# jviquerat/beacon

Measured on AMD Instinct MI355X. Metric: aggregate env steps/sec, rayleigh-v0 batch=512/GPU 128x64, higher is better.
Workload: dtype f32

## Files before the change

beacon_amd/csrc/jit/ns2d_jit.hip:

```cpp
#if BCN_JIT_ROWS == 1 && BCN_JIT_KIND != 0
#error "ns2d_fast_impl.h (one row per lane, ny <= 64) implements the rayleigh boundary conditions only: mixing needs BCN_JIT_ROWS=2"
#endif
#if BCN_JIT_ROWS == 1
#include "../ns2d_fast_impl.h"
#elif BCN_JIT_ROWS == 2
#include "../ns2d_fast2_impl.h"
#else
#include "../ns2d_fast4_impl.h"
#endif

#ifndef BCN_JIT_GF
#define BCN_JIT_GF 0
#endif

extern "C" {

__attribute__((visibility("default"))) int bcn_jit_launch(const void* args, int batch, void* stream) {
#ifdef BCN_JIT_BREAK
#ifndef BCN_JIT_BREAK_EPS
#define BCN_JIT_BREAK_EPS 3e-4
#endif
  NS2DArgs<BCN_JIT_REAL> a = *static_cast<const NS2DArgs<BCN_JIT_REAL>*>(args);
#if BCN_JIT_BREAK == 2
  a.dt *= BCN_JIT_REAL(1.0 + BCN_JIT_BREAK_EPS);
#else
  a.dt *= BCN_JIT_REAL(1.5);
#endif
#else
  const NS2DArgs<BCN_JIT_REAL>& a = *static_cast<const NS2DArgs<BCN_JIT_REAL>*>(args);
#endif
  if (a.nx != BCN_JIT_NX || a.ny != BCN_JIT_NY || a.kind != BCN_JIT_KIND) {
    bcn_set_error("kernel plugin built for %dx%d kind %d, handle is %dx%d kind %d", BCN_JIT_NX, BCN_JIT_NY, BCN_JIT_KIND,
                  a.nx, a.ny, a.kind);
    return BCN_ERR_ARG;
  }
#if BCN_JIT_ROWS == 1
  return launch_fast<BCN_JIT_REAL, BCN_JIT_NX, BCN_JIT_NY, BCN_JIT_R, BCN_JIT_KIND, BCN_JIT_GF>(a, batch, static_cast<hipStream_t>(stream));
#elif BCN_JIT_ROWS == 2
  return launch_fast2<BCN_JIT_REAL, BCN_JIT_NX, BCN_JIT_NY, BCN_JIT_R, BCN_JIT_KIND, BCN_JIT_GF>(a, batch, static_cast<hipStream_t>(stream));
#else
  return launch_fast4<BCN_JIT_REAL, BCN_JIT_NX, BCN_JIT_NY, BCN_JIT_R, BCN_JIT_RPL, BCN_JIT_KIND>(a, batch, static_cast<hipStream_t>(stream));
#endif
}

__attribute__((visibility("default"))) size_t bcn_jit_scratch_elems(void) {
#if BCN_JIT_ROWS == 1
  return FastGeom<BCN_JIT_NX, BCN_JIT_NY, BCN_JIT_R, BCN_JIT_GF>::scratch_elems();
#elif BCN_JIT_ROWS == 2
  return Fast2Geom<BCN_JIT_NX, BCN_JIT_NY, BCN_JIT_R, BCN_JIT_GF>::scratch_elems();
#else
  return 0;
#endif
}

__attribute__((visibility("default"))) size_t bcn_jit_lds_bytes(void) {
#if BCN_JIT_ROWS == 1
  return FastGeom<BCN_JIT_NX, BCN_JIT_NY, BCN_JIT_R, BCN_JIT_GF>::lds_bytes<BCN_JIT_REAL>();
#elif BCN_JIT_ROWS == 2
  return Fast2Geom<BCN_JIT_NX, BCN_JIT_NY, BCN_JIT_R, BCN_JIT_GF>::lds_elems() * sizeof(BCN_JIT_REAL);
#else
  return (size_t)Fast4Geom<BCN_JIT_NX, BCN_JIT_NY, BCN_JIT_R, BCN_JIT_RPL>::lds_elems(sizeof(BCN_JIT_REAL)) * sizeof(BCN_JIT_REAL);
#endif
}

}
```

beacon_amd/csrc/ns2d_fast_impl.h:

```cpp
#pragma once
#include <stdlib.h>

#include <type_traits>

#include "bcn_dpp.h"
#include "ns2d.h"
#include "ns2d_device.h"
#include "ns2d_sched.h"


#ifndef BCN_R128
#define BCN_R128 16
#endif
#ifndef BCN_R50
#define BCN_R50 5
#endif
#ifndef BCN_GFD
#define BCN_GFD 2
#endif
#ifndef BCN_PDG
#define BCN_PDG 8
#endif
static_assert(BCN_PDG == 4 || BCN_PDG == 8 || BCN_PDG == 10 || BCN_PDG == 12 || BCN_PDG == 16 || BCN_PDG == 20,
              "BCN_PDG: only the prefetch depths that were measured AND verified against the oracle (4, 8, 10, 12, 16, 20)");
#ifndef BCN_PDF
#define BCN_PDF 8
#endif
#ifndef BCN_R128D
#define BCN_R128D 16
#endif



namespace {

using namespace bcn_dpp;

template <int NX, int NY, int R, int GF = 0>
struct FastGeom {
  static_assert(NY <= 64, "lanes run along y");
  static constexpr int NW = (NX + R - 1) / R;
  static constexpr int RL = NX - (NW - 1) * R;
  static_assert(NW <= 16 && RL >= 3 && RL <= R, "at most 16 waves, at least 3 columns each");
  static constexpr int NT = NW * 64;
  static constexpr int SY = NY + 2;
  static constexpr int SX = NX + 2;
  static constexpr int DEADPAD = (GF == 2 && RL != R) ? (R - RL + 2) * SY : 0;
  static constexpr int SZ = (SX * SY + 16 + DEADPAD + 63) / 64 * 64;
  static constexpr int PD = GF ? BCN_PDG : BCN_PDF;
  static constexpr int XC = (GF == 2) ? 2 : 4;
  static constexpr int EXCH = 2 * NW * XC * 64;
  static constexpr int MISC = EXCH + 224 + 16;
  static constexpr int FRONT = ((MISC > 63 * SY + 1 ? MISC : 63 * SY + 1) + 15) / 16 * 16;
  static constexpr int BACK = (NY + 3 * PD + 2) * SY;
  static constexpr int FRONTG = (63 * SY + 1 + 15) / 16 * 16;
  static constexpr int MISCA = (MISC + 15) / 16 * 16;
  static constexpr size_t base_elems() {
    return GF == 1 ? (size_t)MISCA : GF == 2 ? (size_t)MISCA + 2 * (size_t)SZ : (size_t)FRONT + 3 * (size_t)SZ + BACK;
  }
  static constexpr size_t SCR = 3 * (size_t)R * 64;
  template <typename real> static constexpr bool offload() {
    return NW >= 3 && (R + 3) / 4 <= NW - 1 && (base_elems() + SCR) * sizeof(real) <= 160 * 1024;
  }
  template <typename real> static constexpr size_t lds_bytes() {
    return (base_elems() + (offload<real>() ? SCR : 0)) * sizeof(real);
  }
  static constexpr size_t scratch_elems() {
    return GF == 1 ? (size_t)FRONTG + 3 * (size_t)SZ + BACK : GF == 2 ? (size_t)FRONTG + SZ + BACK : 0;
  }
};

typedef float v2f __attribute__((ext_vector_type(2)));
#ifndef BCN_CHAIN_NOP
#define BCN_CHAIN_NOP "s_nop 0\n\t"
#endif
template <int NX, int NY, int R>
__device__ __attribute__((noinline)) void transport_chain_f32(float* Tl, const float* Ul, float* dummy, float c0x, float c1x,
                                                              float c0y, float c1y) {
  using G = FastGeom<NX, NY, R, 0>;
  constexpr int SY = G::SY, PD = G::PD, NSTEP = NX + NY - 1;
  static_assert(PD % 2 == 0, "blocks of an even number of diagonals (packed coefficient fmas)");
  const int lane = threadIdx.x & 63;
  const int j = lane + 1;
  const bool active = lane < NY;
  const int cb = (1 - lane) * SY + j;
  float* Tb = Tl + cb;
  for (int i = 1 + lane; i <= NX; i += 64) Tl[i * SY + 1] += (c0y + c1y * Ul[i * SY + 1 + G::SZ]) * Tl[i * SY];
  float tp = Tl[0 * SY + j];
  float aA[PD], uA[PD], vA[PD], aB[PD], uB[PD], vB[PD];
  typedef __attribute__((address_space(3))) float lds_f;
  lds_f* Tc = (lds_f*)Tb;
  const lds_f* Uc = (const lds_f*)(Ul + cb);
  lds_f* const dummyL = (lds_f*)dummy;
#define BCN_LOAD(RA, RU, RV, OFF)                                                             \
  {                                                                                           \
    const lds_f* const Tq = Tc + (OFF) * SY;                                                  \
    const lds_f* const Uq = Uc + (OFF) * SY;                                                  \
    const lds_f* const Vq = Uq + G::SZ;                                                       \
    _Pragma("unroll") for (int q = 0; q < PD; q++) { RA[q] = Tq[q * SY]; RU[q] = Uq[q * SY]; RV[q] = Vq[q * SY]; } \
  }
#define BCN_BLOCK(RA, RU, RV, NA, NU, NV, OFF, MASK)                                          \
  {                                                                                           \
    BCN_LOAD(NA, NU, NV, (OFF) + PD)                                                          \
    lds_f* const Tq = Tc + (OFF) * SY;                                                        \
    float tq[PD];                                                                             \
    bool okq[PD];                                                                             \
     \
    v2f awp[PD / 2], asp[PD / 2];                                                             \
    _Pragma("unroll") for (int q = 0; q < PD / 2; q++) {                                      \
      const v2f ru = {RU[2 * q], RU[2 * q + 1]}, rv = {RV[2 * q], RV[2 * q + 1]};             \
      awp[q] = c0x + c1x * ru;                                                                \
      asp[q] = c0y + c1y * rv;                                                                \
    }                                                                                         \
    _Pragma("unroll") for (int q = 0; q < PD; q++) {                                          \
      const int t = t0 + (OFF) + q;                                                           \
      const float aw = awp[q / 2][q & 1], as = asp[q / 2][q & 1];                             \
      float t1 = RA[q] + aw * tp;                                                             \
      asm volatile(BCN_CHAIN_NOP "v_fmac_f32_dpp %0, %1, %2 wave_shr:1 row_mask:0xf bank_mask:0xf" \
                   : "+v"(t1) : "v"(tp), "v"(as));                                            \
      okq[q] = (MASK == 0) || (MASK == 4 ? (lane <= t) : (active && (MASK != 2 ? (lane <= t) : true) && \
                               (MASK != 1 ? (lane > t - NX && t < NSTEP) : true)));           \
      tp = okq[q] ? t1 : tp;                                                                  \
                  \
      tq[q] = (MASK == 4 && !okq[q]) ? RA[q] : t1;                                            \
    }                                                                                         \
    if (MASK == 0 || MASK == 4) {                                                             \
      _Pragma("unroll") for (int q = 0; q < PD; q++) Tq[q * SY] = tq[q];                      \
    } else {                                                                                  \
      _Pragma("unroll") for (int q = 0; q < PD; q++) { lds_f* dst = okq[q] ? Tq + q * SY : dummyL; *dst = tq[q]; } \
    }                                                                                         \
  }
#define BCN_CHAIN2(T0, T1, MASK)                                                              \
  _Pragma("nounroll") for (int t0 = (T0); t0 < (T1); t0 += 2 * PD) {                          \
    BCN_BLOCK(aA, uA, vA, aB, uB, vB, 0, MASK)                                                \
    BCN_BLOCK(aB, uB, vB, aA, uA, vA, PD, MASK)                                               \
    Tc += 2 * PD * SY;                                                                        \
    Uc += 2 * PD * SY;                                                                        \
  }
  BCN_LOAD(aA, uA, vA, 0)
  constexpr int P2 = 2 * PD;
  constexpr int TA2 = ((NY - 1 + P2 - 1) / P2) * P2, TB2 = (NX / P2) * P2, TE2 = ((NSTEP + P2 - 1) / P2) * P2;
  if constexpr (TA2 <= TB2 && NY == 64) {
    const float east = Tl[(NX + 1) * SY + j];
    BCN_CHAIN2(0, TA2, 4)
    BCN_CHAIN2(TA2, TE2, 0)
    Tl[(NX + 1) * SY + j] = east;
  } else {
    BCN_CHAIN2(0, TE2, 3)
  }
#undef BCN_CHAIN2
#undef BCN_BLOCK
#undef BCN_LOAD
}

template <typename real, int NX, int NY, int R, int GF>
__device__ __attribute__((noinline)) void transport_chain(real* Tl, const real* Ul, const real* Vl, real* dummy,
                                                          real c0x, real c1x, real c0y, real c1y) {
  using G = FastGeom<NX, NY, R, GF>;
  constexpr int SY = G::SY, PD = G::PD, NSTEP = NX + NY - 1;
  const int lane = threadIdx.x & 63;
  const int j = lane + 1;
  const bool active = lane < NY;
  const int cb = (1 - lane) * SY + j;
  typedef typename std::conditional<GF != 0, __attribute__((address_space(1))) real, __attribute__((address_space(3))) real>::type treal;
  typedef typename std::conditional<GF == 1, __attribute__((address_space(1))) real, __attribute__((address_space(3))) real>::type ureal;
  treal* const Tb = (treal*)(Tl + cb);
  treal* const dummy_t = GF != 0 ? (treal*)(Tl - G::FRONTG) : (treal*)dummy;
  const ureal* const Ug = (const ureal*)Ul;
  const ureal* const Vg = (const ureal*)Vl;
  auto ldu = [&](int t) -> real { const int x = cb + t * SY; return GF == 2 ? Ug[x < 0 ? 0 : (x >= G::SZ ? G::SZ - 1 : x)] : Ug[x]; };
  auto ldv = [&](int t) -> real { const int x = cb + t * SY; return GF == 2 ? Vg[x < 0 ? 0 : (x >= G::SZ ? G::SZ - 1 : x)] : Vg[x]; };
  for (int i = 1 + lane; i <= NX; i += 64) {
    const int x = i * SY + 1;
    ((treal*)Tl)[x] = ((treal*)Tl)[x] + (c0y + c1y * Vg[x]) * ((treal*)Tl)[x - 1];
  }
  asm volatile("s_waitcnt vmcnt(0) lgkmcnt(0)" ::: "memory");
  real ra[PD], ru[PD], rv[PD];
#pragma unroll
  for (int q = 0; q < PD; q++) { ra[q] = Tb[q * SY]; ru[q] = ldu(q); rv[q] = ldv(q); }
  real tp = Tl[0 * SY + j];
#define BCN_CHAIN(T0, T1, MASK)                                                             \
// ... 6 lines not shown
      if (MASK == 0) {                                                                      \
        tp = tn;                                                                            \
        Tb[t * SY] = tn;                                                                    \
      } else {                                                                              \
        const bool ok = active && (MASK != 2 ? (lane <= t) : true) &&                       \
                        (MASK != 1 ? (lane > t - NX && t < NSTEP) : true);                  \
        tp = ok ? tn : tp;                                                                  \
        treal* dst = ok ? Tb + t * SY : dummy_t;                                            \
        *dst = tn;                                                                          \
      }                                                                                     \
      ra[q] = Tb[(t + PD) * SY];                                                            \
      ru[q] = ldu(t + PD);                                                                  \
      rv[q] = ldv(t + PD);                                                                  \
    }                                                                                       \
  }
  constexpr int TA = ((NY - 1 + PD - 1) / PD) * PD;
  constexpr int TB = (NX / PD) * PD;
  if constexpr (TA <= TB) {
    BCN_CHAIN(0, TA, 1)
    if (NY == 64) { BCN_CHAIN(TA, TB, 0) } else { BCN_CHAIN(TA, TB, 1) }
    BCN_CHAIN(TB, NSTEP, 2)
  } else {
    constexpr int TL = ((NY - 1) / PD) * PD, TH = ((NX + PD - 1) / PD) * PD;
    BCN_CHAIN(0, TL, 1)
    BCN_CHAIN(TL, TH, 3)
    BCN_CHAIN(TH, NSTEP, 2)
  }
#undef BCN_CHAIN
}

template <typename real, int NX, int NY, int R0, int RW, int KIND, bool EQ, int GF>
__device__ __forceinline__ void fast_body(const NS2DArgs<real>& A, const int w, const int b, const int it_begin, const int it_end,
                                          const bool first_chunk, const bool last_chunk, char* smem) {
  using G = FastGeom<NX, NY, R0, GF>;
  constexpr int R = RW;
  constexpr int NW = G::NW, NT = G::NT, SY = G::SY, SX = G::SX, SZ = G::SZ, PD = G::PD;
  real* exch = reinterpret_cast<real*>(smem);
  real* errp = exch + G::EXCH;
  real* sact = errp + 128;
  real* red = sact + 64;
  real* gscr = GF ? A.fscr + (size_t)blockIdx.x * A.fscr_stride + G::FRONTG : nullptr;
  real* Ul = GF == 1 ? gscr : GF == 2 ? exch + G::MISCA : exch + G::FRONT;
  real* Vl = Ul + SZ;
  real* Tl = GF == 2 ? gscr : Vl + SZ;

  const int tid = threadIdx.x, lane = tid & 63;
  int j = lane + 1;
  const bool active = lane < NY;
  constexpr int RL = G::RL;
  constexpr bool DEADC = GF == 2 && RW == R0 && RL != R0;
  static_assert(!(DEADC && G::XC == 4), "dead columns exist only in the single-sweep exchange paths (XC == 2, GF == 2)");
  const bool lastw = DEADC && w == NW - 1;
#define LIVE(k) (!DEADC || (k) < RL || !lastw)
  const int i0 = w * R0 + 1;
  const size_t off = (size_t)b * A.ncell;
  real* __restrict__ gu = A.u + off;
  real* __restrict__ gv = A.v + off;
  real* __restrict__ gp = A.p + off;
  real* __restrict__ gS = A.S + off;
  constexpr int XC = G::XC, XL = XC - 1;
  auto exl = [&](int buf, int wave, int which) -> real& { return exch[((buf * NW + wave) * XC + which) * 64 + lane]; };

  for (int c = tid; c < SX * SY; c += NT) {
    const int jj = c / SX, ii = c - jj * SX;
    Ul[ii * SY + jj] = gu[c];
    Vl[ii * SY + jj] = gv[c];
    Tl[ii * SY + jj] = gS[c];
  }
  for (int c = SX * SY + tid; c < SZ; c += NT) { Ul[c] = 0; Vl[c] = 0; Tl[c] = 0; }
  if (tid < 128) errp[tid] = 0;
  real p[R];
#pragma unroll
  for (int k = 0; k < R; k++) p[k] = (active && LIVE(k)) ? gp[j * SX + i0 + k] : real(0);

  if (!first_chunk) {
    if (tid < A.n_sgts) sact[tid] = A.a_last[(size_t)b * A.n_sgts + tid];
  } else {
    const int n = A.n_sgts;
    const real* src = A.actions ? A.actions + (size_t)b * n : A.a_last + (size_t)b * n;
    real mean = 0;
    for (int k = 0; k < n; k++) mean += src[k];
    mean /= (real)n;
    real m = 1;
    for (int k = 0; k < n; k++) {
      real t = bcn_abs(src[k] - mean) / A.C;
      m = t > m ? t : m;
    }
    real mine = (tid < n) ? (src[tid] - mean) / m : real(0);
    __syncthreads();
    if (tid < n) {
      sact[tid] = mine;
      A.a_last[(size_t)b * n + tid] = mine;
      if (A.actions_norm) A.actions_norm[(size_t)b * n + tid] = mine;
    }
  }
  __syncthreads();

  const real dt = A.dt, rdx = A.rdx, rdy = A.rdy, rdx2 = A.rdx2, rdy2 = A.rdy2;
  const real cx = A.cx, cy = A.cy;
  const real wl = active ? real(1) + (j == 1 ? 1 : 0) + ((j == NY && KIND == 0) ? 1 : 0) : real(0);
  const real fW = (active && w == 0) ? real(1) : real(0);
  const real fE = (active && w == NW - 1) ? real(1) : real(0);
// ... 27 lines not shown
  if (tid == 0) {
    slow_k[0] = 0; slow_k[5] = 0;
    slow_k[1] = (real)A.slow_l2lc[0]; slow_k[2] = (real)A.slow_cl[0];
    slow_k[3] = (real)A.slow_l2lc[1]; slow_k[4] = (real)A.slow_cl[1];
  }

  constexpr bool OFFLOAD = G::template offload<real>();
  real* const P0 = exch + G::base_elems();
  real* const US0 = P0 + R0 * 64;
  real* const VX0 = US0 + R0 * 64;
  auto pred = [&](const int i, real uc, real uE_, real uW_, real uN_, real uS_, real uSE_, real vc, real vE_, real vW_, real vN_,
                  real vS_, real vNW_, real pc, real pW, real pS, real& us_out, real& vx_out) {
    {
      real uE = real(0.5) * (uE_ + uc), uW = real(0.5) * (uc + uW_);
      real uN2 = real(0.5) * (uN_ + uc), uS2 = real(0.5) * (uc + uS_);
      real vN2 = real(0.5) * (vN_ + vNW_), vS2 = real(0.5) * (vc + vW_);
      real conv = (uE * uE - uW * uW) * rdx + (uN2 * vN2 - uS2 * vS2) * rdy;
      real diff = ((uE_ - 2 * uc + uW_) * rdx2 + (uN_ - 2 * uc + uS_) * rdy2) * A.kmom;
      real pres = (pc - pW) * rdx;
      us_out = (i >= 2 && (!DEADC || i <= NX) && active) ? uc + dt * (diff - conv - pres) : real(0);
    }
    {
      real vE = real(0.5) * (vE_ + vc), vW = real(0.5) * (vc + vW_);
      real uE = real(0.5) * (uE_ + uSE_), uW = real(0.5) * (uc + uS_);
      real vN2 = real(0.5) * (vN_ + vc), vS2 = real(0.5) * (vc + vS_);
      real conv = (uE * vE - uW * vW) * rdx + (vN2 * vN2 - vS2 * vS2) * rdy;
      real diff = ((vE_ - 2 * vc + vW_) * rdx2 + (vN_ - 2 * vc + vS_) * rdy2) * A.kmom;
      real pres = (pc - pS) * rdy;
      vx_out = diff - conv - pres;
    }
  };
  auto bc_uv = [&]() {
    for (int jj = 1 + tid; jj <= NY; jj += NT) {
      Ul[1 * SY + jj] = 0;
      Ul[(NX + 1) * SY + jj] = 0;
      if (jj >= 2) {
        Vl[0 * SY + jj] = -Vl[1 * SY + jj];
        Vl[(NX + 1) * SY + jj] = -Vl[NX * SY + jj];
      }
    }
    for (int ii = 1 + tid; ii <= NX + 1; ii += NT) {
      const bool wall = (ii == 1) || (ii == NX + 1);
      const real utop = wall ? real(0) : Ul[ii * SY + NY];
      const real ubot = wall ? real(0) : Ul[ii * SY + 1];
      Ul[ii * SY + NY + 1] = -utop;
      Ul[ii * SY + 0] = -ubot;
      if (ii <= NX) {
        Vl[ii * SY + NY + 1] = 0;
        Vl[ii * SY + 1] = 0;
      }
    }
  };
  auto publish_p = [&]() {
    exl(xb, w, 1) = p[R - 1];
    if (OFFLOAD && w == 0) {
#pragma unroll
      for (int k = 0; k < R; k++) P0[k * 64 + lane] = p[k];
    }
  };

  bc_uv();
  publish_p();
  __syncthreads();

  real us[R], vs[R];
  for (int it = it_begin;; it++) {
    asm volatile("" : "+v"(j));
    const bool have_chain = it > it_begin;
    const bool have_pred = it < it_end && status == 0;
    real vx[R];
    const bool pred_own = have_pred && (w != 0 || !have_chain);
    if (w == 0 && have_chain) {
#ifndef BCN_CHAIN_PRIO
#define BCN_CHAIN_PRIO 3
#endif
      __builtin_amdgcn_s_setprio(BCN_CHAIN_PRIO);
      if constexpr (std::is_same<real, float>::value && GF == 0)
        transport_chain_f32<NX, NY, R0>(Tl, Ul, red + 16, dt * A.ksc * rdx2, real(0.5) * dt * rdx, dt * A.ksc * rdy2,
                                        real(0.5) * dt * rdy);
      else
        transport_chain<real, NX, NY, R0, GF>(Tl, Ul, Vl, red + 16, dt * A.ksc * rdx2, real(0.5) * dt * rdx,
                                              dt * A.ksc * rdy2, real(0.5) * dt * rdy);
      __builtin_amdgcn_s_setprio(0);
      BCN_PH(6)
    }
#define BCN_OWN_PRED                                                                                            \
    {                                                                                                           \
      const real pWh = (w > 0) ? exl(xb, w - 1, 1) : real(0);                                              \
       \
      constexpr bool WIDE = (R > 16) || (R > 12 && NW > 8);    \
      constexpr int CH = GF ? 4 : (!WIDE ? R : (R % 4 == 0 ? 4 : 5));    \
      _Pragma("unroll") for (int c0 = 0; c0 < R; c0 += CH) {                                                    \
        if (CH != R) __builtin_amdgcn_sched_barrier(0);           \
        real ur[CH + 2], uS[CH + 1], uN[CH], vr[CH + 2], vN[CH + 1], vS[CH];                                    \
        const int ic = i0 + c0;                                                                                 \
        _Pragma("unroll") for (int k = 0; k < CH + 2; k++) { ur[k] = Ul[(ic - 1 + k) * SY + j]; vr[k] = Vl[(ic - 1 + k) * SY + j]; } \
        _Pragma("unroll") for (int k = 0; k < CH + 1; k++) { uS[k] = Ul[(ic + k) * SY + j - 1]; vN[k] = Vl[(ic - 1 + k) * SY + j + 1]; } \
        _Pragma("unroll") for (int k = 0; k < CH; k++) { uN[k] = Ul[(ic + k) * SY + j + 1]; vS[k] = Vl[(ic + k) * SY + j - 1]; } \
        _Pragma("unroll") for (int k = 0; k < CH; k++) {                                                        \
          const int kk = c0 + k;                                                                                \
          if (kk >= R) continue;                                \
          const real pc = p[kk < R ? kk : 0];                                                                   \
          const real pW = (kk > 0) ? p[kk > 0 && kk <= R ? kk - 1 : 0] : pWh;                                   \
          const real pS = from_below(pc, pc);                                                                   \
          pred(ic + k, ur[k + 1], ur[k + 2], ur[k], uN[k], uS[k], uS[k + 1], vr[k + 1], vr[k + 2], vr[k], vN[k + 1], vS[k], \
               vN[k], pc, pW, pS, us[kk < R ? kk : 0], vx[kk < R ? kk : 0]);                                    \
        }                                                                                                       \
      }                                                                                                         \
    }
    if (pred_own) BCN_OWN_PRED
    if constexpr (OFFLOAD) {
      if (have_pred && have_chain && w != 0) {
        constexpr int CH0 = 4, NCH0 = (R0 + CH0 - 1) / CH0;
        static_assert(NCH0 <= NW - 1, "one chunk of strip 0 per helper wave");
        const int c = (NW == 8) ? (w < 4 ? w - 1 : (w == 4 ? 6 : w - 2)) : w - 1;
        if (c < NCH0) {
          const int kc = c * CH0;
          real ur[CH0 + 2], uS[CH0 + 1], uN[CH0], vr[CH0 + 2], vN[CH0 + 1], vS[CH0], pp[CH0 + 1];
          const int ic = 1 + kc;
#pragma unroll
          for (int k = 0; k < CH0 + 2; k++) { ur[k] = Ul[(ic - 1 + k) * SY + j]; vr[k] = Vl[(ic - 1 + k) * SY + j]; }
#pragma unroll
          for (int k = 0; k < CH0 + 1; k++) { uS[k] = Ul[(ic + k) * SY + j - 1]; vN[k] = Vl[(ic - 1 + k) * SY + j + 1]; }
#pragma unroll
          for (int k = 0; k < CH0; k++) { uN[k] = Ul[(ic + k) * SY + j + 1]; vS[k] = Vl[(ic + k) * SY + j - 1]; }
#pragma unroll
          for (int k = 0; k <= CH0; k++) {
            const int kk = kc + k - 1;
            const int kq = kk < 0 ? 0 : (kk < R0 ? kk : R0 - 1);
            const real pv = P0[kq * 64 + lane];
            pp[k] = (kk >= 0 && kk < R0) ? pv : real(0);
          }
#pragma unroll
          for (int k = 0; k < CH0; k++) {
            const int kk = kc + k;
            const real pc = pp[k + 1];
            const real pS = from_below(pc, pc);
            real uo, xo;
            pred(ic + k, ur[k + 1], ur[k + 2], ur[k], uN[k], uS[k], uS[k + 1], vr[k + 1], vr[k + 2], vr[k], vN[k + 1], vS[k], vN[k],
                 pc, pp[k], pS, uo, xo);
            if (kk < R0) {
              US0[kk * 64 + lane] = uo;
              VX0[kk * 64 + lane] = xo;
            }
          }
        }
      }
    }
    if (w != 0) { BCN_PH(6) }
    if (have_pred) xb ^= 1;
    if (have_pred && w != 0) exl(xb, w, 0) = us[0];
    __syncthreads();
    BCN_PH(5)
    if (!have_pred) break;
    asm volatile("" : "+v"(j));
    if (w == 0 && have_chain) {
      if constexpr (OFFLOAD) {
#pragma unroll
        for (int k = 0; k < R; k++) { us[k] = US0[k * 64 + lane]; vx[k] = VX0[k * 64 + lane]; }
      } else {
        BCN_OWN_PRED
      }
    }
#undef BCN_OWN_PRED
    constexpr bool TREG = GF == 2 && KIND == 0;
    real Tr[TREG ? R : 1];
    if constexpr (TREG) {
#pragma unroll
      for (int k = 0; k < R; k++) Tr[k] = Tl[(i0 + k) * SY + j];
      if (active) {
        if (w == 0) Tl[0 * SY + j] = Tr[0];
        if (w == NW - 1) Tl[(NX + 1) * SY + j] = Tr[(DEADC ? RL : R) - 1];
      }
      {
        real gt = 0, gb = 0;
#pragma unroll
        for (int k = 0; k < R; k++) {
          const real tt = read_lane(Tr[k], NY - 1), tb = read_lane(Tr[k], 0);
          gt = (lane == k) ? 2 * A.Tc - tt : gt;
          gb = (lane == k) ? tb : gb;
        }
        const int ii = i0 + (lane < R ? lane : 0);
        const int sg = (ii - 1) / A.nx_sgts;
        const real sa = sact[sg < A.n_sgts ? sg : 0];
        if (lane < (lastw ? RL : R)) {
          Tl[ii * SY + NY + 1] = gt;
          if (sg < A.n_sgts) Tl[ii * SY + 0] = 2 * (A.Th + sa) - gb;
        }
      }
    } else {
    for (int jj = 1 + tid; jj <= NY; jj += NT) {
      Tl[0 * SY + jj] = Tl[1 * SY + jj];
      Tl[(NX + 1) * SY + jj] = Tl[NX * SY + jj];
    }
    for (int ii = 1 + tid; ii <= NX; ii += NT) {
      Tl[ii * SY + NY + 1] = 2 * A.Tc - Tl[ii * SY + NY];
      const int k = (ii - 1) / A.nx_sgts;
      if (k < A.n_sgts) Tl[ii * SY + 0] = 2 * (A.Th + sact[k]) - Tl[ii * SY + 1];
    }
    }
#pragma unroll
    for (int k = 0; k < R; k++) {
      const real buoy = (KIND == 0) ? (TREG ? Tr[TREG ? k : 0] : Tl[(i0 + k) * SY + j]) : real(0);
      vs[k] = (j >= 2 && active && LIVE(k)) ? Vl[(i0 + k) * SY + j] + dt * (vx[k] + buoy) : real(0);
    }
    BCN_PH(0)

    real nb[R];
    {
      const real usE = (w < NW - 1) ? exl(xb, w + 1, 0) : real(0);
      xb ^= 1;
#pragma unroll
      for (int k = 0; k < R; k++) {
        const real ue = (k < R - 1) ? us[k < R - 1 ? k + 1 : 0] : usE;
        const real vn = from_above(real(0), vs[k]);
        nb[k] = (active && LIVE(k)) ? -A.cb * ((ue - us[k]) * rdx + (vn - vs[k]) * rdy) : real(0);
      }
    }
    const int wm = (w > 0) ? w - 1 : 0, wp = (w < NW - 1) ? w + 1 : NW - 1;
    real nbW = 0, nbE = 0;
    if constexpr (XC == 4) {
      exl(xb, w, 0) = nb[0];
      exl(xb, w, 3) = nb[R - 1];
      real a1p = 0;
#pragma unroll
      for (int k = 0; k < R; k++) a1p += nb[k] * nb[k];
      const real a1w = wave_sum_lane63<real>(a1p);
      if (lane == 63) exch[((xb * NW + w) * XC + 1) * 64] = a1w;
      __syncthreads();
      nbW = exl(xb, wm, 3);
      nbE = exl(xb, wp, 0);
      const real a1q = (lane < NW) ? exch[((xb * NW + (lane < NW ? lane : 0)) * XC + 1) * 64] : real(0);
      const real a1 = read_lane(row16_sum<real>(a1q), 15);
      if (tid == 0) slow_k[0] = (real)(0.5f * __log2f(3.f * (float)a1 / (float)A.tol));
      xb ^= 1;
    } else if (A.conv_plan == 3) {
      real a1p = 0;
// ... 341 lines not shown
      }
      if (tid == 0) { prev_sweeps[0] = 0; prev_sweeps[1] = toofar ? real(0) : real(1); prev_sweeps[3] += 1; }
      __syncthreads();
    }
    }
    if (finalB) {
#pragma unroll
      for (int k = 0; k < R; k++) phA[k] = phB[k];
    }
    hW = hW1r;
#ifdef BCN_STAMP
    {
      const unsigned long long st1 = __builtin_amdgcn_s_memtime();
      const int cps = (int)((st1 - st0) / (unsigned long long)(itp > 0 ? itp : 1));
      if (A.sweeps && tid == 0) A.sweeps[(size_t)b * A.ndt_act + it] = itp | (cps << 16);
    }
#elif defined(BCN_DBG_NCHK)
    if (A.sweeps && tid == 0) A.sweeps[(size_t)b * A.ndt_act + it] = itp | (nchk << 16);
#else
    if (A.sweeps && tid == 0) A.sweeps[(size_t)b * A.ndt_act + it] = itp;
#endif

    cyc_j += __builtin_amdgcn_s_memtime() - cyc_j0;
    asm volatile("" : "+v"(j));
    BCN_PH(2)
#pragma unroll
    for (int k = 0; k < R; k++) {
      const int i = i0 + k;
      const real ph = phA[k];
      const real pw = (k > 0) ? phA[k > 0 ? k - 1 : 0] : hW;
      const real ps = from_below(ph, ph);
      p[k] += ph;
      if (active) {
        if (i >= 2 && LIVE(k)) Ul[i * SY + j] = us[k] - dt * (ph - pw) * rdx;
        if (j >= 2 && LIVE(k)) Vl[i * SY + j] = vs[k] - dt * (ph - ps) * rdy;
      }
    }
    __syncthreads();

    asm volatile("" : "+v"(j));
    BCN_PH(3)
    {
      real Ac[R];
      real Tx[TREG ? R + 1 : 1];
      if constexpr (TREG) {
#pragma unroll
        for (int k = 0; k <= R; k++) Tx[k] = Tl[(i0 + k) * SY + j];
      }
#pragma unroll
      for (int k = 0; k < R; k++) {
        const int c = (i0 + k) * SY + j;
        const real uE = Ul[c + SY], uW = Ul[c], vN = Vl[c + 1], vS = Vl[c];
        real T0, TE, TN;
        if constexpr (TREG) {
          T0 = Tx[TREG ? k : 0]; TE = Tx[TREG ? k + 1 : 0];
          TN = from_above(real(0), T0);
          TN = (lane == NY - 1) ? 2 * A.Tc - T0 : TN;
        } else {
          T0 = Tl[c]; TE = Tl[c + SY]; TN = Tl[c + 1];
        }
        const real expl = A.ksc * ((TE - 2 * T0) * rdx2 + (TN - 2 * T0) * rdy2) -
                          (uE * real(0.5) * (TE + T0) - uW * real(0.5) * T0) * rdx -
                          (vN * real(0.5) * (TN + T0) - vS * real(0.5) * T0) * rdy;
        Ac[k] = T0 + dt * expl;
      }
      if (it + 1 < it_end && status == 0) {
        bc_uv();
        publish_p();
      }
      __syncthreads();
      if (active) {
#pragma unroll
        for (int k = 0; k < R; k++) if (LIVE(k)) Tl[(i0 + k) * SY + j] = Ac[k];
      }
    }
    __syncthreads();
    BCN_PH(4)
  }
#undef BCN_NCHK_INC

  for (int c = tid; c < SX * SY; c += NT) {
    const int jj = c / SX, ii = c - jj * SX;
    gu[c] = Ul[ii * SY + jj];
    gv[c] = Vl[ii * SY + jj];
    gS[c] = Tl[ii * SY + jj];
  }
  if (active) {
#pragma unroll
    for (int k = 0; k < R; k++) {
      const int i = i0 + k, c = j * SX + i;
      if (!LIVE(k)) continue;
      const real dp = p[k] - gp[c];
      if (i == 1) gp[c - 1] += dp;
      if (i == NX) gp[c + 1] += dp;
      if (j == 1) gp[c - SX] += dp;
      if (j == NY && KIND == 0) gp[c + SX] += dp;
      gp[c] = p[k];
    }
  }
  __syncthreads();
#ifdef BCN_STAMP
  {
    const unsigned long long kt1 = __builtin_amdgcn_s_memtime(), kr1 = __builtin_amdgcn_s_memrealtime();
    status = (int)((kt1 - kt0) * 100ull / (kr1 - kr0 + 1));
#ifndef BCN_STAMP_WAVE
#define BCN_STAMP_WAVE 0
#endif
    if (tid == 64 * BCN_STAMP_WAVE && A.actions_norm)
      for (int q = 0; q < 7; q++) A.actions_norm[(size_t)b * A.n_sgts + q] = (real)seg[q] / (real)(it_end - it_begin);

  }
#endif
  if (last_chunk) {
    ns2d_finish<real, NT>(A, b, gu, gv, gS, status, red);
  } else if (tid == 0) {
    A.status[b] = status;
  }
#undef LIVE
  if (tid == 0 && A.cyc) {
    A.cyc[4 * (size_t)b] += cyc_j;
    A.cyc[4 * (size_t)b + 1] += __builtin_amdgcn_s_memtime() - cyc_u0;
    A.cyc[4 * (size_t)b + 2] += (unsigned long long)prev_sweeps[2];
    A.cyc[4 * (size_t)b + 3] += (unsigned long long)prev_sweeps[3];
  }
}

template <typename real, int NX, int NY, int R, int KIND, bool EQ, int GF>
__device__ __forceinline__ void fast_unit(const NS2DArgs<real>& A, const int b, const int it_begin, const int it_end,
                                          const bool first_chunk, const bool last_chunk, char* smem) {
  using G = FastGeom<NX, NY, R, GF>;
  const int w = __builtin_amdgcn_readfirstlane(threadIdx.x >> 6);
  if (GF != 2 && G::RL != R && w == G::NW - 1) fast_body<real, NX, NY, R, G::RL, KIND, EQ, GF>(A, w, b, it_begin, it_end, first_chunk, last_chunk, smem);
  else fast_body<real, NX, NY, R, R, KIND, EQ, GF>(A, w, b, it_begin, it_end, first_chunk, last_chunk, smem);
}

template <typename real, int NX, int NY, int R, int KIND, bool EQ, int GF>
__global__ __launch_bounds__((FastGeom<NX, NY, R, GF>::NT)) void ns2d_fast_step(NS2DArgs<real> A) {
  extern __shared__ __attribute__((aligned(16))) char smem[];
  const int b = A.order ? A.order[blockIdx.x] : (int)blockIdx.x;
  if (A.mask && !A.mask[b]) return;
  fast_unit<real, NX, NY, R, KIND, EQ, GF>(A, b, A.it_begin, A.it_end, A.first_chunk != 0, A.last_chunk != 0, smem);
}

template <typename real, int NX, int NY, int R, int KIND, bool EQ, int GF>
__global__ __launch_bounds__((FastGeom<NX, NY, R, GF>::NT)) void ns2d_fast_sched(NS2DArgs<real> A, SchedCtl* ctl, int batch, int nchunk) {
  extern __shared__ __attribute__((aligned(16))) char smem[];
  unsigned int* s_words = reinterpret_cast<unsigned int*>(reinterpret_cast<real*>(smem) +
                                                          FastGeom<NX, NY, R, GF>::EXCH + 224);
  ns2d_sched_loop<real>(A, ctl, batch, nchunk, s_words, [&](int b, int it0, int it1, bool first, bool last) {
    fast_unit<real, NX, NY, R, KIND, EQ, GF>(A, b, it0, it1, first, last, smem);
  });
}

__global__ __launch_bounds__(1024) void ns2d_rank_by_work(const int32_t* sweeps, int ndt, int q, int batch,
                                                          int32_t* order, const uint8_t* mask) {
  __shared__ int key[2048];
  for (int b = threadIdx.x; b < batch; b += blockDim.x) {
    int s = 0;
    if (!mask || mask[b])
      for (int t = 0; t < q; t++) s += sweeps[(size_t)b * ndt + t];
    key[b] = s;
  }
  __syncthreads();
  for (int b = threadIdx.x; b < batch; b += blockDim.x) {
    const int mine = key[b];
    int rank = 0;
    for (int o = 0; o < batch; o++) rank += (key[o] > mine || (key[o] == mine && o < b)) ? 1 : 0;
    order[rank] = b;
  }
}

template <typename real, int NX, int NY, int R, int KIND, bool EQ, int GF>
int launch_fast_eq(const NS2DArgs<real>& a, int batch, hipStream_t s) {
  using G = FastGeom<NX, NY, R, GF>;
  if (GF && (!a.fscr || a.fscr_stride < G::scratch_elems())) { bcn_set_error("fast path: field scratch missing"); return BCN_ERR_UNSUPPORTED; }
  const size_t lds = G::template lds_bytes<real>();
  auto k = ns2d_fast_step<real, NX, NY, R, KIND, EQ, GF>;
  static unsigned long long attr_set = 0;
  if (ns2d_first_on_device(attr_set)) {
    BCN_HIP(hipFuncSetAttribute(reinterpret_cast<const void*>(k), hipFuncAttributeMaxDynamicSharedMemorySize, (int)lds));
  }
  NS2DArgs<real> c = a;
  if (!c.sweeps) c.sweeps = c.sweeps_int;
  const SchedParams sp = ns2d_sched_params(a);
  const int mode = sp.mode, sched_grid = sp.grid, SQ = sp.q;
  if (mode == 2 && batch > sched_grid && a.ndt_act >= 2 * SQ && a.sched_ctl) {
    auto ks = ns2d_fast_sched<real, NX, NY, R, KIND, EQ, GF>;
    static unsigned long long attr_set2 = 0;
    if (ns2d_first_on_device(attr_set2)) {
      BCN_HIP(hipFuncSetAttribute(reinterpret_cast<const void*>(ks), hipFuncAttributeMaxDynamicSharedMemorySize, (int)lds));
    }
    int nchunk = 0;
    ns2d_sched_chunks(a.ndt_act, SQ, (a.host ? a.host->sched_tail : 0), &c.sched_nbig, &nchunk);
    c.sched_q = SQ; c.order = nullptr; c.first_chunk = 1; c.last_chunk = 1; c.it_begin = 0; c.it_end = a.ndt_act;
    BCN_HIP(hipMemsetAsync(a.sched_ctl, 0, a.sched_bytes, s));
    hipLaunchKernelGGL(ks, dim3(sched_grid), dim3(G::NT), lds, s, c, static_cast<SchedCtl*>(a.sched_ctl), batch, nchunk);
    BCN_HIP(hipGetLastError());
    if (a.host) a.host->launched = "ns2d_fast_sched";
    return BCN_OK;
  }
  const int min_batch = sp.lpt_min_batch;
  constexpr int Q = 10;
  const bool split = mode >= 1 && batch >= min_batch && batch <= 2048 && a.ndt_act >= 4 * Q;
  c.first_chunk = 1; c.order = nullptr; c.it_begin = 0;
  if (a.sched_ctl) BCN_HIP(hipMemsetAsync(a.sched_ctl, 0, a.sched_bytes, s));
  if (!split) {
    c.it_end = a.ndt_act; c.last_chunk = 1;
// ... 23 lines not shown
```

Before: 29650.

## Store LDS fields row-major so the transport sweep uses 16-byte vector accesses

For f32 fields held in LDS, the grid layout changes from column-major (stride SY along x) to row-major with a padded pitch P ≡ 1 mod 4. The diagonal transport wave then steps by one element per diagonal and can load and store through aligned 16-byte LDS vectors, which replaces the scalar strided accesses and the masked dummy-address stores. The prefetch depth grows to BCN_PDR and the chain mask logic is reworked so masked cells write back their old value. Every other LDS index in the kernel goes through an accessor macro, which changes the bank patterns of the other phases and adds LDS padding.

```diff
diff --git a/beacon_amd/csrc/jit/ns2d_jit.hip b/beacon_amd/csrc/jit/ns2d_jit.hip
--- a/beacon_amd/csrc/jit/ns2d_jit.hip
+++ b/beacon_amd/csrc/jit/ns2d_jit.hip
@@ -55,7 +55,7 @@
 
 __attribute__((visibility("default"))) size_t bcn_jit_lds_bytes(void) {
 #if BCN_JIT_ROWS == 1
-  return FastGeom<BCN_JIT_NX, BCN_JIT_NY, BCN_JIT_R, BCN_JIT_GF>::lds_bytes<BCN_JIT_REAL>();
+  return FastGeomF<BCN_JIT_REAL, BCN_JIT_NX, BCN_JIT_NY, BCN_JIT_R, BCN_JIT_GF>::lds_bytes<BCN_JIT_REAL>();
 #elif BCN_JIT_ROWS == 2
   return Fast2Geom<BCN_JIT_NX, BCN_JIT_NY, BCN_JIT_R, BCN_JIT_GF>::lds_elems() * sizeof(BCN_JIT_REAL);
 #else
diff --git a/beacon_amd/csrc/ns2d_fast_impl.h b/beacon_amd/csrc/ns2d_fast_impl.h
--- a/beacon_amd/csrc/ns2d_fast_impl.h
+++ b/beacon_amd/csrc/ns2d_fast_impl.h
@@ -26,6 +26,9 @@
 #ifndef BCN_PDF
 #define BCN_PDF 8
 #endif
+#ifndef BCN_PDR
+#define BCN_PDR 16
+#endif
 #ifndef BCN_R128D
 #define BCN_R128D 16
 #endif
@@ -36,23 +39,36 @@
 
 using namespace bcn_dpp;
 
-template <int NX, int NY, int R, int GF = 0>
+template <int NX, int NY, int R, int GF = 0, bool RM = false>
 struct FastGeom {
   static_assert(NY <= 64, "lanes run along y");
+  static_assert(!RM || GF == 0, "the row-major layout is for fields in LDS");
+  static constexpr bool ROWMAJOR = RM;
   static constexpr int NW = (NX + R - 1) / R;
   static constexpr int RL = NX - (NW - 1) * R;
   static_assert(NW <= 16 && RL >= 3 && RL <= R, "at most 16 waves, at least 3 columns each");
   static constexpr int NT = NW * 64;
   static constexpr int SY = NY + 2;
   static constexpr int SX = NX + 2;
+  static constexpr int P = SX + (5 - SX % 4) % 4;
+  static_assert(P % 4 == 1 && P >= SX, "row pitch");
+  static constexpr int O = RM ? 2 : 0;
+  static constexpr int XS = RM ? 1 : SY;
+  static constexpr int YS = RM ? P : 1;
+  static __host__ __device__ constexpr int at(int i, int j) { return O + i * XS + j * YS; }
   static constexpr int DEADPAD = (GF == 2 && RL != R) ? (R - RL + 2) * SY : 0;
-  static constexpr int SZ = (SX * SY + 16 + DEADPAD + 63) / 64 * 64;
-  static constexpr int PD = GF ? BCN_PDG : BCN_PDF;
+  static constexpr int SZ = RM ? (O + SY * P + 63) / 64 * 64 : (SX * SY + 16 + DEADPAD + 63) / 64 * 64;
+  static constexpr int PD = GF ? BCN_PDG : (RM && SX + (5 - SX % 4) % 4 - 1 >= 2 * BCN_PDR) ? BCN_PDR : BCN_PDF;
   static constexpr int XC = (GF == 2) ? 2 : 4;
   static constexpr int EXCH = 2 * NW * XC * 64;
   static constexpr int MISC = EXCH + 224 + 16;
-  static constexpr int FRONT = ((MISC > 63 * SY + 1 ? MISC : 63 * SY + 1) + 15) / 16 * 16;
-  static constexpr int BACK = (NY + 3 * PD + 2) * SY;
+  static constexpr int TE2 = (NX + NY - 1 + 2 * PD - 1) / (2 * PD) * (2 * PD);
+  static constexpr int RDEND_CHAIN = O + P + 1 + 63 * (P - 1) + TE2 + PD;
+  static constexpr int RDEND_ROWS = O + 66 * P;
+  static constexpr int RDEND = RDEND_CHAIN > RDEND_ROWS ? RDEND_CHAIN : RDEND_ROWS;
+  static constexpr int FRONT = RM ? (MISC + 15) / 16 * 16 : ((MISC > 63 * SY + 1 ? MISC : 63 * SY + 1) + 15) / 16 * 16;
+  static constexpr int BACK = RM ? (RDEND > SZ ? (RDEND - SZ + 15) / 16 * 16 : 0)
+                                 : (NY + 3 * PD + 2) * SY;
   static constexpr int FRONTG = (63 * SY + 1 + 15) / 16 * 16;
   static constexpr int MISCA = (MISC + 15) / 16 * 16;
   static constexpr size_t base_elems() {
@@ -68,43 +84,48 @@
   static constexpr size_t scratch_elems() {
     return GF == 1 ? (size_t)FRONTG + 3 * (size_t)SZ + BACK : GF == 2 ? (size_t)FRONTG + SZ + BACK : 0;
   }
+  static_assert(!RM || (FRONT % 4 == 0 && SZ % 64 == 0 && (O + P + 1) % 4 == 0 && (P - 1) % 4 == 0),
+                "row-major: the transport wave's 16-byte vectors are aligned for every lane");
+  static_assert(!RM || P - 1 >= 2 * PD, "row-major: a cell the transport wave reaches twice (two lanes, P - 1 steps apart) is "
+                                           "stored back long after the other visit's load");
+  static_assert(!RM || lds_bytes<float>() <= 160 * 1024, "LDS");
 };
+template <typename real, int NX, int NY, int R, int GF>
+using FastGeomF = FastGeom<NX, NY, R, GF, std::is_same<real, float>::value && GF == 0>;
 
 typedef float v2f __attribute__((ext_vector_type(2)));
+typedef float v4f __attribute__((ext_vector_type(4)));
 #ifndef BCN_CHAIN_NOP
 #define BCN_CHAIN_NOP "s_nop 0\n\t"
 #endif
 template <int NX, int NY, int R>
-__device__ __attribute__((noinline)) void transport_chain_f32(float* Tl, const float* Ul, float* dummy, float c0x, float c1x,
-                                                              float c0y, float c1y) {
-  using G = FastGeom<NX, NY, R, 0>;
-  constexpr int SY = G::SY, PD = G::PD, NSTEP = NX + NY - 1;
-  static_assert(PD % 2 == 0, "blocks of an even number of diagonals (packed coefficient fmas)");
+__device__ __attribute__((noinline)) void transport_chain_f32(float* Tl, const float* Ul, float c0x, float c1x, float c0y,
+                                                              float c1y) {
+  using G = FastGeom<NX, NY, R, 0, true>;
+  constexpr int PD = G::PD, SZ = G::SZ;
+  static_assert(PD % 4 == 0, "blocks of whole 16-byte vectors");
   const int lane = threadIdx.x & 63;
   const int j = lane + 1;
   const bool active = lane < NY;
-  const int cb = (1 - lane) * SY + j;
-  float* Tb = Tl + cb;
-  for (int i = 1 + lane; i <= NX; i += 64) Tl[i * SY + 1] += (c0y + c1y * Ul[i * SY + 1 + G::SZ]) * Tl[i * SY];
-  float tp = Tl[0 * SY + j];
+  for (int i = 1 + lane; i <= NX; i += 64) Tl[G::at(i, 1)] += (c0y + c1y * Ul[G::at(i, 1) + SZ]) * Tl[G::at(i, 0)];
+  float tp = Tl[G::at(0, j)];
   float aA[PD], uA[PD], vA[PD], aB[PD], uB[PD], vB[PD];
   typedef __attribute__((address_space(3))) float lds_f;
-  lds_f* Tc = (lds_f*)Tb;
+  typedef __attribute__((address_space(3))) v4f lds_v4;
+  const int cb = G::at(1 - lane, j);
+  lds_f* Tc = (lds_f*)(Tl + cb);
   const lds_f* Uc = (const lds_f*)(Ul + cb);
-  lds_f* const dummyL = (lds_f*)dummy;
 #define BCN_LOAD(RA, RU, RV, OFF)                                                             \
-  {                                                                                           \
-    const lds_f* const Tq = Tc + (OFF) * SY;                                                  \
-    const lds_f* const Uq = Uc + (OFF) * SY;                                                  \
-    const lds_f* const Vq = Uq + G::SZ;                                                       \
-    _Pragma("unroll") for (int q = 0; q < PD; q++) { RA[q] = Tq[q * SY]; RU[q] = Uq[q * SY]; RV[q] = Vq[q * SY]; } \
+  _Pragma("unroll") for (int q = 0; q < PD; q += 4) {                                         \
+    const v4f a = *(const lds_v4*)(Tc + (OFF) + q), u = *(const lds_v4*)(Uc + (OFF) + q),     \
+              v = *(const lds_v4*)(Uc + (OFF) + q + SZ);                                      \
+    _Pragma("unroll") for (int k = 0; k < 4; k++) { RA[q + k] = a[k]; RU[q + k] = u[k]; RV[q + k] = v[k]; } \
   }
 #define BCN_BLOCK(RA, RU, RV, NA, NU, NV, OFF, MASK)                                          \
   {                                                                                           \
     BCN_LOAD(NA, NU, NV, (OFF) + PD)                                                          \
-    lds_f* const Tq = Tc + (OFF) * SY;                                                        \
+    lds_f* const Tq = Tc + (OFF);                                                             \
     float tq[PD];                                                                             \
-    bool okq[PD];                                                                             \
      \
     v2f awp[PD / 2], asp[PD / 2];                                                             \
     _Pragma("unroll") for (int q = 0; q < PD / 2; q++) {                                      \
@@ -115,38 +136,35 @@
     _Pragma("unroll") for (int q = 0; q < PD; q++) {                                          \
       const int t = t0 + (OFF) + q;                                                           \
       const float aw = awp[q / 2][q & 1], as = asp[q / 2][q & 1];                             \
-      float t1 = RA[q] + aw * tp;                                                             \
-      asm volatile(BCN_CHAIN_NOP "v_fmac_f32_dpp %0, %1, %2 wave_shr:1 row_mask:0xf bank_mask:0xf" \
-                   : "+v"(t1) : "v"(tp), "v"(as));                                            \
-      okq[q] = (MASK == 0) || (MASK == 4 ? (lane <= t) : (active && (MASK != 2 ? (lane <= t) : true) && \
-                               (MASK != 1 ? (lane > t - NX && t < NSTEP) : true)));           \
-      tp = okq[q] ? t1 : tp;                                                                  \
-                  \
-      tq[q] = (MASK == 4 && !okq[q]) ? RA[q] : t1;                                            \
+      float t1;                                                                               \
+      asm volatile("v_fma_f32 %0, %1, %2, %3\n\t" BCN_CHAIN_NOP                               \
+                   "v_fmac_f32_dpp %0, %1, %4 wave_shr:1 row_mask:0xf bank_mask:0xf"          \
+                   : "=&v"(t1) : "v"(tp), "v"(aw), "v"(RA[q]), "v"(as));                      \
+      const bool inF = !((MASK) & 1) || lane <= t;                                            \
+      const bool ok = inF && (!((MASK) & 2) || lane > t - NX) && (!((MASK) & 4) || active);  \
+      tp = ((MASK) & 1) ? (inF ? t1 : tp) : t1;                                               \
+      tq[q] = (MASK) ? (ok ? t1 : RA[q]) : t1;                                                \
     }                                                                                         \
-    if (MASK == 0 || MASK == 4) {                                                             \
-      _Pragma("unroll") for (int q = 0; q < PD; q++) Tq[q * SY] = tq[q];                      \
-    } else {                                                                                  \
-      _Pragma("unroll") for (int q = 0; q < PD; q++) { lds_f* dst = okq[q] ? Tq + q * SY : dummyL; *dst = tq[q]; } \
-    }                                                                                         \
+    _Pragma("unroll") for (int q = 0; q < PD; q += 4)                                         \
+      *(lds_v4*)(Tq + q) = v4f{tq[q], tq[q + 1], tq[q + 2], tq[q + 3]};                       \
   }
 #define BCN_CHAIN2(T0, T1, MASK)                                                              \
   _Pragma("nounroll") for (int t0 = (T0); t0 < (T1); t0 += 2 * PD) {                          \
     BCN_BLOCK(aA, uA, vA, aB, uB, vB, 0, MASK)                                                \
     BCN_BLOCK(aB, uB, vB, aA, uA, vA, PD, MASK)                                               \
-    Tc += 2 * PD * SY;                                                                        \
-    Uc += 2 * PD * SY;                                                                        \
+    Tc += 2 * PD;                                                                             \
+    Uc += 2 * PD;                                                                             \
   }
   BCN_LOAD(aA, uA, vA, 0)
-  constexpr int P2 = 2 * PD;
-  constexpr int TA2 = ((NY - 1 + P2 - 1) / P2) * P2, TB2 = (NX / P2) * P2, TE2 = ((NSTEP + P2 - 1) / P2) * P2;
-  if constexpr (TA2 <= TB2 && NY == 64) {
-    const float east = Tl[(NX + 1) * SY + j];
-    BCN_CHAIN2(0, TA2, 4)
-    BCN_CHAIN2(TA2, TE2, 0)
-    Tl[(NX + 1) * SY + j] = east;
+  constexpr int P2 = 2 * PD, RW = NY < 64 ? 4 : 0;
+  constexpr int TA2 = ((NY - 1 + P2 - 1) / P2) * P2, TB2 = (NX / P2) * P2, TE2 = G::TE2;
+  static_assert(TE2 >= NX + NY - 1, "the sweep");
+  if constexpr (TA2 <= TB2) {
+    BCN_CHAIN2(0, TA2, 1 | RW)
+    BCN_CHAIN2(TA2, TB2, RW)
+    BCN_CHAIN2(TB2, TE2, 2 | RW)
   } else {
-    BCN_CHAIN2(0, TE2, 3)
+    BCN_CHAIN2(0, TE2, 3 | RW)
   }
 #undef BCN_CHAIN2
 #undef BCN_BLOCK
@@ -219,7 +237,7 @@
 template <typename real, int NX, int NY, int R0, int RW, int KIND, bool EQ, int GF>
 __device__ __forceinline__ void fast_body(const NS2DArgs<real>& A, const int w, const int b, const int it_begin, const int it_end,
                                           const bool first_chunk, const bool last_chunk, char* smem) {
-  using G = FastGeom<NX, NY, R0, GF>;
+  using G = FastGeomF<real, NX, NY, R0, GF>;
   constexpr int R = RW;
   constexpr int NW = G::NW, NT = G::NT, SY = G::SY, SX = G::SX, SZ = G::SZ, PD = G::PD;
   real* exch = reinterpret_cast<real*>(smem);
@@ -230,6 +248,7 @@
   real* Ul = GF == 1 ? gscr : GF == 2 ? exch + G::MISCA : exch + G::FRONT;
   real* Vl = Ul + SZ;
   real* Tl = GF == 2 ? gscr : Vl + SZ;
+#define BCN_AT(I, J) (G::ROWMAJOR ? G::at(I, J) : (I) * SY + J)
 
   const int tid = threadIdx.x, lane = tid & 63;
   int j = lane + 1;
@@ -248,13 +267,24 @@
   constexpr int XC = G::XC, XL = XC - 1;
   auto exl = [&](int buf, int wave, int which) -> real& { return exch[((buf * NW + wave) * XC + which) * 64 + lane]; };
 
+  if constexpr (G::ROWMAJOR) {
+    for (int c = tid; c < SZ; c += NT) {
+      const int e = c - G::O, jj = e / G::P, ii = e - jj * G::P;
+      real u = 0, v = 0, t = 0;
+      if (e >= 0 && jj < SY && ii < SX) { u = gu[jj * SX + ii]; v = gv[jj * SX + ii]; t = gS[jj * SX + ii]; }
+      Ul[c] = u;
+      Vl[c] = v;
+      Tl[c] = t;
+    }
+  } else {
   for (int c = tid; c < SX * SY; c += NT) {
     const int jj = c / SX, ii = c - jj * SX;
-    Ul[ii * SY + jj] = gu[c];
-    Vl[ii * SY + jj] = gv[c];
-    Tl[ii * SY + jj] = gS[c];
+    Ul[BCN_AT(ii, jj)] = gu[c];
+    Vl[BCN_AT(ii, jj)] = gv[c];
+    Tl[BCN_AT(ii, jj)] = gS[c];
   }
   for (int c = SX * SY + tid; c < SZ; c += NT) { Ul[c] = 0; Vl[c] = 0; Tl[c] = 0; }
+  }
   if (tid < 128) errp[tid] = 0;
   real p[R];
 #pragma unroll
@@ -348,22 +378,22 @@
   };
   auto bc_uv = [&]() {
     for (int jj = 1 + tid; jj <= NY; jj += NT) {
-      Ul[1 * SY + jj] = 0;
-      Ul[(NX + 1) * SY + jj] = 0;
+      Ul[BCN_AT(1, jj)] = 0;
+      Ul[BCN_AT(NX + 1, jj)] = 0;
       if (jj >= 2) {
-        Vl[0 * SY + jj] = -Vl[1 * SY + jj];
-        Vl[(NX + 1) * SY + jj] = -Vl[NX * SY + jj];
+        Vl[BCN_AT(0, jj)] = -Vl[BCN_AT(1, jj)];
+        Vl[BCN_AT(NX + 1, jj)] = -Vl[BCN_AT(NX, jj)];
       }
     }
     for (int ii = 1 + tid; ii <= NX + 1; ii += NT) {
       const bool wall = (ii == 1) || (ii == NX + 1);
-      const real utop = wall ? real(0) : Ul[ii * SY + NY];
-      const real ubot = wall ? real(0) : Ul[ii * SY + 1];
-      Ul[ii * SY + NY + 1] = -utop;
-      Ul[ii * SY + 0] = -ubot;
+      const real utop = wall ? real(0) : Ul[BCN_AT(ii, NY)];
+      const real ubot = wall ? real(0) : Ul[BCN_AT(ii, 1)];
+      Ul[BCN_AT(ii, NY + 1)] = -utop;
+      Ul[BCN_AT(ii, 0)] = -ubot;
       if (ii <= NX) {
-        Vl[ii * SY + NY + 1] = 0;
-        Vl[ii * SY + 1] = 0;
+        Vl[BCN_AT(ii, NY + 1)] = 0;
+        Vl[BCN_AT(ii, 1)] = 0;
       }
     }
   };
@@ -392,8 +422,7 @@
 #endif
       __builtin_amdgcn_s_setprio(BCN_CHAIN_PRIO);
       if constexpr (std::is_same<real, float>::value && GF == 0)
-        transport_chain_f32<NX, NY, R0>(Tl, Ul, red + 16, dt * A.ksc * rdx2, real(0.5) * dt * rdx, dt * A.ksc * rdy2,
-                                        real(0.5) * dt * rdy);
+        transport_chain_f32<NX, NY, R0>(Tl, Ul, dt * A.ksc * rdx2, real(0.5) * dt * rdx, dt * A.ksc * rdy2, real(0.5) * dt * rdy);
       else
         transport_chain<real, NX, NY, R0, GF>(Tl, Ul, Vl, red + 16, dt * A.ksc * rdx2, real(0.5) * dt * rdx,
                                               dt * A.ksc * rdy2, real(0.5) * dt * rdy);
@@ -410,9 +439,9 @@
         if (CH != R) __builtin_amdgcn_sched_barrier(0);           \
         real ur[CH + 2], uS[CH + 1], uN[CH], vr[CH + 2], vN[CH + 1], vS[CH];                                    \
         const int ic = i0 + c0;                                                                                 \
-        _Pragma("unroll") for (int k = 0; k < CH + 2; k++) { ur[k] = Ul[(ic - 1 + k) * SY + j]; vr[k] = Vl[(ic - 1 + k) * SY + j]; } \
-        _Pragma("unroll") for (int k = 0; k < CH + 1; k++) { uS[k] = Ul[(ic + k) * SY + j - 1]; vN[k] = Vl[(ic - 1 + k) * SY + j + 1]; } \
-        _Pragma("unroll") for (int k = 0; k < CH; k++) { uN[k] = Ul[(ic + k) * SY + j + 1]; vS[k] = Vl[(ic + k) * SY + j - 1]; } \
+        _Pragma("unroll") for (int k = 0; k < CH + 2; k++) { ur[k] = Ul[BCN_AT(ic - 1 + k, j)]; vr[k] = Vl[BCN_AT(ic - 1 + k, j)]; } \
+        _Pragma("unroll") for (int k = 0; k < CH + 1; k++) { uS[k] = Ul[BCN_AT(ic + k, j - 1)]; vN[k] = Vl[BCN_AT(ic - 1 + k, j + 1)]; } \
+        _Pragma("unroll") for (int k = 0; k < CH; k++) { uN[k] = Ul[BCN_AT(ic + k, j + 1)]; vS[k] = Vl[BCN_AT(ic + k, j - 1)]; } \
         _Pragma("unroll") for (int k = 0; k < CH; k++) {                                                        \
           const int kk = c0 + k;                                                                                \
           if (kk >= R) continue;                                \
@@ -435,11 +464,11 @@
           real ur[CH0 + 2], uS[CH0 + 1], uN[CH0], vr[CH0 + 2], vN[CH0 + 1], vS[CH0], pp[CH0 + 1];
           const int ic = 1 + kc;
 #pragma unroll
-          for (int k = 0; k < CH0 + 2; k++) { ur[k] = Ul[(ic - 1 + k) * SY + j]; vr[k] = Vl[(ic - 1 + k) * SY + j]; }
-#pragma unroll
-          for (int k = 0; k < CH0 + 1; k++) { uS[k] = Ul[(ic + k) * SY + j - 1]; vN[k] = Vl[(ic - 1 + k) * SY + j + 1]; }
-#pragma unroll
-          for (int k = 0; k < CH0; k++) { uN[k] = Ul[(ic + k) * SY + j + 1]; vS[k] = Vl[(ic + k) * SY + j - 1]; }
+          for (int k = 0; k < CH0 + 2; k++) { ur[k] = Ul[BCN_AT(ic - 1 + k, j)]; vr[k] = Vl[BCN_AT(ic - 1 + k, j)]; }
+#pragma unroll
+          for (int k = 0; k < CH0 + 1; k++) { uS[k] = Ul[BCN_AT(ic + k, j - 1)]; vN[k] = Vl[BCN_AT(ic - 1 + k, j + 1)]; }
+#pragma unroll
+          for (int k = 0; k < CH0; k++) { uN[k] = Ul[BCN_AT(ic + k, j + 1)]; vS[k] = Vl[BCN_AT(ic + k, j - 1)]; }
 #pragma unroll
           for (int k = 0; k <= CH0; k++) {
             const int kk = kc + k - 1;
@@ -483,10 +512,10 @@
     real Tr[TREG ? R : 1];
     if constexpr (TREG) {
 #pragma unroll
-      for (int k = 0; k < R; k++) Tr[k] = Tl[(i0 + k) * SY + j];
+      for (int k = 0; k < R; k++) Tr[k] = Tl[BCN_AT(i0 + k, j)];
       if (active) {
-        if (w == 0) Tl[0 * SY + j] = Tr[0];
-        if (w == NW - 1) Tl[(NX + 1) * SY + j] = Tr[(DEADC ? RL : R) - 1];
+        if (w == 0) Tl[BCN_AT(0, j)] = Tr[0];
+        if (w == NW - 1) Tl[BCN_AT(NX + 1, j)] = Tr[(DEADC ? RL : R) - 1];
       }
       {
         real gt = 0, gb = 0;
@@ -500,25 +529,25 @@
         const int sg = (ii - 1) / A.nx_sgts;
         const real sa = sact[sg < A.n_sgts ? sg : 0];
         if (lane < (lastw ? RL : R)) {
-          Tl[ii * SY + NY + 1] = gt;
-          if (sg < A.n_sgts) Tl[ii * SY + 0] = 2 * (A.Th + sa) - gb;
+          Tl[BCN_AT(ii, NY + 1)] = gt;
+          if (sg < A.n_sgts) Tl[BCN_AT(ii, 0)] = 2 * (A.Th + sa) - gb;
         }
       }
     } else {
     for (int jj = 1 + tid; jj <= NY; jj += NT) {
-      Tl[0 * SY + jj] = Tl[1 * SY + jj];
-      Tl[(NX + 1) * SY + jj] = Tl[NX * SY + jj];
+      Tl[BCN_AT(0, jj)] = Tl[BCN_AT(1, jj)];
+      Tl[BCN_AT(NX + 1, jj)] = Tl[BCN_AT(NX, jj)];
     }
     for (int ii = 1 + tid; ii <= NX; ii += NT) {
-      Tl[ii * SY + NY + 1] = 2 * A.Tc - Tl[ii * SY + NY];
+      Tl[BCN_AT(ii, NY + 1)] = 2 * A.Tc - Tl[BCN_AT(ii, NY)];
       const int k = (ii - 1) / A.nx_sgts;
-      if (k < A.n_sgts) Tl[ii * SY + 0] = 2 * (A.Th + sact[k]) - Tl[ii * SY + 1];
+      if (k < A.n_sgts) Tl[BCN_AT(ii, 0)] = 2 * (A.Th + sact[k]) - Tl[BCN_AT(ii, 1)];
     }
     }
 #pragma unroll
     for (int k = 0; k < R; k++) {
-      const real buoy = (KIND == 0) ? (TREG ? Tr[TREG ? k : 0] : Tl[(i0 + k) * SY + j]) : real(0);
-      vs[k] = (j >= 2 && active && LIVE(k)) ? Vl[(i0 + k) * SY + j] + dt * (vx[k] + buoy) : real(0);
+      const real buoy = (KIND == 0) ? (TREG ? Tr[TREG ? k : 0] : Tl[BCN_AT(i0 + k, j)]) : real(0);
+      vs[k] = (j >= 2 && active && LIVE(k)) ? Vl[BCN_AT(i0 + k, j)] + dt * (vx[k] + buoy) : real(0);
     }
     BCN_PH(0)
 
@@ -926,8 +955,8 @@
       const real ps = from_below(ph, ph);
       p[k] += ph;
       if (active) {
-        if (i >= 2 && LIVE(k)) Ul[i * SY + j] = us[k] - dt * (ph - pw) * rdx;
-        if (j >= 2 && LIVE(k)) Vl[i * SY + j] = vs[k] - dt * (ph - ps) * rdy;
+        if (i >= 2 && LIVE(k)) Ul[BCN_AT(i, j)] = us[k] - dt * (ph - pw) * rdx;
+        if (j >= 2 && LIVE(k)) Vl[BCN_AT(i, j)] = vs[k] - dt * (ph - ps) * rdy;
       }
     }
     __syncthreads();
@@ -939,19 +968,19 @@
       real Tx[TREG ? R + 1 : 1];
       if constexpr (TREG) {
 #pragma unroll
-        for (int k = 0; k <= R; k++) Tx[k] = Tl[(i0 + k) * SY + j];
+        for (int k = 0; k <= R; k++) Tx[k] = Tl[BCN_AT(i0 + k, j)];
       }
 #pragma unroll
       for (int k = 0; k < R; k++) {
-        const int c = (i0 + k) * SY + j;
-        const real uE = Ul[c + SY], uW = Ul[c], vN = Vl[c + 1], vS = Vl[c];
+        const int c = BCN_AT((i0 + k), j);
+        const real uE = Ul[c + G::XS], uW = Ul[c], vN = Vl[c + G::YS], vS = Vl[c];
         real T0, TE, TN;
         if constexpr (TREG) {
           T0 = Tx[TREG ? k : 0]; TE = Tx[TREG ? k + 1 : 0];
           TN = from_above(real(0), T0);
           TN = (lane == NY - 1) ? 2 * A.Tc - T0 : TN;
         } else {
-          T0 = Tl[c]; TE = Tl[c + SY]; TN = Tl[c + 1];
+          T0 = Tl[c]; TE = Tl[c + G::XS]; TN = Tl[c + G::YS];
         }
         const real expl = A.ksc * ((TE - 2 * T0) * rdx2 + (TN - 2 * T0) * rdy2) -
                           (uE * real(0.5) * (TE + T0) - uW * real(0.5) * T0) * rdx -
@@ -965,7 +994,7 @@
       __syncthreads();
       if (active) {
 #pragma unroll
-        for (int k = 0; k < R; k++) if (LIVE(k)) Tl[(i0 + k) * SY + j] = Ac[k];
+        for (int k = 0; k < R; k++) if (LIVE(k)) Tl[BCN_AT(i0 + k, j)] = Ac[k];
       }
     }
     __syncthreads();
@@ -975,9 +1004,9 @@
 
   for (int c = tid; c < SX * SY; c += NT) {
     const int jj = c / SX, ii = c - jj * SX;
-    gu[c] = Ul[ii * SY + jj];
-    gv[c] = Vl[ii * SY + jj];
-    gS[c] = Tl[ii * SY + jj];
+    gu[c] = Ul[BCN_AT(ii, jj)];
+    gv[c] = Vl[BCN_AT(ii, jj)];
+    gS[c] = Tl[BCN_AT(ii, jj)];
   }
   if (active) {
 #pragma unroll
@@ -1017,6 +1046,7 @@
     A.cyc[4 * (size_t)b + 2] += (unsigned long long)prev_sweeps[2];
     A.cyc[4 * (size_t)b + 3] += (unsigned long long)prev_sweeps[3];
   }
+#undef BCN_AT
 }
 
 template <typename real, int NX, int NY, int R, int KIND, bool EQ, int GF>
@@ -1066,7 +1096,7 @@
 
 template <typename real, int NX, int NY, int R, int KIND, bool EQ, int GF>
 int launch_fast_eq(const NS2DArgs<real>& a, int batch, hipStream_t s) {
-  using G = FastGeom<NX, NY, R, GF>;
+  using G = FastGeomF<real, NX, NY, R, GF>;
   if (GF && (!a.fscr || a.fscr_stride < G::scratch_elems())) { bcn_set_error("fast path: field scratch missing"); return BCN_ERR_UNSUPPORTED; }
   const size_t lds = G::template lds_bytes<real>();
   auto k = ns2d_fast_step<real, NX, NY, R, KIND, EQ, GF>;
```

Result: no change. 29760 (median of 6 runs) (+0.4%).
